# simonfuhrmann/mve

Hardware: AMD Instinct MI355X
Metric: depth-maps/sec (1920x1080, 20 views, scale=2) (higher is better)
Workload: dtype f32

## Files before the change

### mve_amd/csrc/dmrecon_device.hip

```cpp
#include <hip/hip_runtime.h>
#include <stdint.h>
#include <cstdlib>
#include <type_traits>

#include "dmrecon_types.h"
#include "dmrecon_device.h"

#define WAVE 64

#ifndef MI_FW
#define MI_FW 5
#endif
#define MI_HALF (MI_FW / 2)
#define MI_NS (MI_FW * MI_FW)
#define MI_MID (MI_NS / 2)
#define MI_STEP_SAMPLE (MI_NS > 12 ? 12 : MI_MID)
#define MI_CAT2(a, b) a##b
#define MI_CAT(a, b) MI_CAT2(a, b)
#define MI_FWNS MI_CAT(mi_fw, MI_FW)
#define MI_BULK_WAVES (MI_FW >= 7 ? 1 : MI_WAVES_PER_SIMD)
#ifdef MI_EMU_LIN48
#define MI_QUAD_WORDS 12
#elif defined(MI_QUAD_RECORDS)
#define MI_QUAD_WORDS 4
// ... 1884 lines not shown
#endif
struct XcdRange {
    unsigned per_x, base, j, jn;
    __device__ __forceinline__ explicit XcdRange(unsigned n_units, bool own_segment = false) {
        const unsigned nx = (gridDim.x % MI_XCDS == 0 && gridDim.x >= MI_XCDS) ? MI_XCDS : 1u;
        per_x = own_segment ? n_units : (n_units + nx - 1) / nx;
        base = own_segment ? 0u : (blockIdx.x % nx) * per_x; j = blockIdx.x / nx; jn = gridDim.x / nx;
    }
    __device__ __forceinline__ bool next(unsigned& unit) {
        if (j >= per_x) return false;
        unit = base + j; j += jn;
        return true;
    }
};

template <class L>
__device__ __forceinline__ void flush_counters(DevCounters* counters, int lane, unsigned n_eval, unsigned n_pass,
                                               unsigned n_patch, unsigned n_filled, unsigned err, int kind) {
    if (L::sub(lane) != 0) { n_eval = 0; n_pass = 0; }
    if (L::vslot(lane) != 0 || L::sub(lane) != 0) { n_patch = 0; n_filled = 0; }
    for (int off = 32; off > 0; off >>= 1) {
        n_eval += __shfl_down(n_eval, off);
        n_pass += __shfl_down(n_pass, off);
        n_patch += __shfl_down(n_patch, off);
        n_filled += __shfl_down(n_filled, off);
        err |= __shfl_down(err, off);
    }
    if (lane == 0) {
        if (n_eval) { atomicAdd(&counters->n_eval, (unsigned long long)n_eval); atomicAdd(&counters->k_eval[kind], (unsigned long long)n_eval); }
        if (n_pass) { atomicAdd(&counters->n_pass, (unsigned long long)n_pass); atomicAdd(&counters->k_pass[kind], (unsigned long long)n_pass);
                      atomicAdd(&counters->k_pass_exec[kind], (unsigned long long)n_pass); }
        if (n_patch) { atomicAdd(&counters->n_patch, (unsigned long long)n_patch); atomicAdd(&counters->k_patch[kind], (unsigned long long)n_patch); }
        if (n_filled) atomicAdd(&counters->n_filled, (unsigned long long)n_filled);
        if (err) atomicOr(&counters->error_flags, err);
    }
}

template <class L, bool FAST, bool SINGLE = FAST, bool SEED = false>
__global__ __launch_bounds__(WAVE) __attribute__((amdgpu_waves_per_eu((L::LAT ? 2 : MI_BULK_WAVES), (L::LAT ? 2 : MI_WAVES_PER_SIMD)))) void k_optimize(OptArgs a) {
    static_assert(SINGLE || !FAST, "the FAST kernel runs one attempt per entry");
    static_assert(!SEED || (SINGLE && !FAST), "the seed launch is the single-attempt form of the general kernel");
    const int lane = threadIdx.x;
    const bool grid8 = gridDim.x % MI_XCDS == 0 && gridDim.x >= MI_XCDS;
    const unsigned seg_n = (a.follow_seg != 0u && grid8) ? MI_XCDS : 1u, seg = blockIdx.x % seg_n;
    const unsigned seg_in_n = (a.follow_seg_in != 0u && grid8) ? MI_XCDS : 1u, seg_in = blockIdx.x % seg_in_n;
    const unsigned n = a.follow_in ? a.follow_in_n[seg_in] : (a.n_work_ptr ? *a.n_work_ptr : a.n_work);
    if (!a.follow_in && (n < a.min_work || n >= a.max_work)) return;
    for (int i = lane; i < 256; i += WAVE) g_lut[i] = a.lut[i];
#ifdef MI_ACTIVITY
    if (lane < 2) g_act[lane] = 0;
// ... 131 lines not shown
        PatchResult r; unsigned ne = 0, np = 0;
        unsigned deferred = 0;
        optimize_patch<L, false, true>(job, a.st, a.views, x, y, hd, hi, hj, hv, lane, r, ne, np, err, a.counters, &deferred);
        if (L::sub(lane) != 0) { ne = 0; np = 0; }
        ne = patch_sum_u<L>(ne); np = patch_sum_u<L>(np);
        if (writer) n_exec += np;
        if (writer) {
            DevSpec o;
            o.conf = r.conf; o.depth = r.depth; o.dzI = r.dzI; o.dzJ = r.dzJ; o.nx = r.nx; o.ny = r.ny; o.nz = r.nz;
            o.views = r.views; o.views_hi = r.views_hi; o.iters = r.iters; o.bc = bc; o.own = own; o.n_eval = ne; o.n_pass = np;
            o.n_cand = n_cand; o.pad = (int32_t)deferred;
            *rec = o;
        }
    }
    for (int off = 32; off > 0; off >>= 1) { err |= __shfl_down(err, off); n_exec += __shfl_down(n_exec, off); }
    if (lane == 0 && err) atomicOr(&a.counters->error_flags, err);
    if (lane == 0 && n_exec) atomicAdd(&a.counters->k_pass_exec[MI_KIND_SPEC], (unsigned long long)n_exec);
}

#define MI_TAIL_WAVES 4
static_assert(MI_TAIL_WAVES <= MI_LAT_SLOTS, "the latency layout's LDS holds one patch per wavefront of a tail workgroup");
#ifndef MI_TAIL_SPEC_WAVES
#define MI_TAIL_SPEC_WAVES 2
#endif
struct TailArgs {
    OptArgs o;
    const DevEntry* prev_work;
    const DevResult* prev_results;
    unsigned* round_work;
};

struct Frozen { float conf; int upd; bool one; };
// ... 130 lines not shown
                o.accepted = 1; o.tried = done;
                a.results[e] = o;
                const bool one = me.one;
                float* dp = one ? job->depth : job->depth1; float* zp = one ? job->dz : job->dz1;
                float* cq = one ? job->conf : job->conf1; float* np = one ? job->normal : job->normal1;
                uint32_t* vp = one ? job->views : job->views1; int32_t* up = one ? job->upd : job->upd1;
                dp[q] = fin.depth; zp[2 * q] = fin.dzI; zp[2 * q + 1] = fin.dzJ;
                np[3 * q] = fin.nx; np[3 * q + 1] = fin.ny; np[3 * q + 2] = fin.nz;
                cq[q] = fin.conf; vp[q] = fin.views; up[q] = a.round;
                if (NV == 8) (one ? job->views_hi : job->views1_hi)[q] = fin.views_hi;
                if (own <= 0.f) { ++n_filled; atomicAdd(const_cast<uint32_t*>(&job->n_filled), 1u); }
            }
        }
        if (SPEC && !single) __syncthreads();
    }
    if (threadIdx.x == 0) {
        if (n_eval) { atomicAdd(&a.counters->n_eval, (unsigned long long)n_eval); atomicAdd(&a.counters->k_eval[MI_KIND_TAIL], (unsigned long long)n_eval); }
        if (n_pass) { atomicAdd(&a.counters->n_pass, (unsigned long long)n_pass); atomicAdd(&a.counters->k_pass[MI_KIND_TAIL], (unsigned long long)n_pass);
                      atomicAdd(&a.counters->k_pass_exec[MI_KIND_TAIL], (unsigned long long)n_pass); }
        if (n_patch) { atomicAdd(&a.counters->n_patch, (unsigned long long)n_patch); atomicAdd(&a.counters->k_patch[MI_KIND_TAIL], (unsigned long long)n_patch); }
        if (n_filled) atomicAdd(&a.counters->n_filled, (unsigned long long)n_filled);
    }
    for (int off = 32; off > 0; off >>= 1) err |= __shfl_down(err, off);
    if (lane == 0 && err) atomicOr(&a.counters->error_flags, err);
}



#ifndef MI_FRONT_WAVES
#define MI_FRONT_WAVES 8
#endif
#define MI_FRONT_QCAP 256
#define MI_FRONT_GRAN 12
static_assert(MI_FRONT_WAVES <= MI_LAT_SLOTS, "the latency layout's LDS holds one patch per wavefront of a front workgroup");
struct FrontArgs {
    OptArgs o;
    DevEntry* work[2];
// ... 367 lines not shown
        __hip_atomic_store(t.host_done + jobi, 1u, __ATOMIC_RELEASE, __HIP_MEMORY_SCOPE_SYSTEM);
    }
    if (tid == 0) {
        if (gave_up) {
            atomicMax(t.job_resume + jobi, ((unsigned long long)(unsigned)round << 32) | ((unsigned long long)n_prev << 1) | (unsigned long long)cur);
            atomicOr(&a.counters->error_flags, 32u);
        } else if (n_prev == 0 || abort || g_fcnt[6] != 0) atomicMax(t.job_resume + jobi, MI_FRONT_DONE);
    }
    if (member != 0) { n_eval = 0; n_pass = 0; n_patch = 0; }
    for (int off2 = 32; off2 > 0; off2 >>= 1) {
        n_eval += __shfl_down(n_eval, off2); n_pass += __shfl_down(n_pass, off2);
        n_patch += __shfl_down(n_patch, off2); n_filled += __shfl_down(n_filled, off2);
        err |= __shfl_down(err, off2); st_att += __shfl_down(st_att, off2);
    }
    if (lane == 0) {
        if (n_eval) { atomicAdd(&a.counters->n_eval, (unsigned long long)n_eval); atomicAdd(&a.counters->k_eval[MI_KIND_FRONT], (unsigned long long)n_eval); }
        if (n_pass) { atomicAdd(&a.counters->n_pass, (unsigned long long)n_pass); atomicAdd(&a.counters->k_pass[MI_KIND_FRONT], (unsigned long long)n_pass);
                      atomicAdd(&a.counters->k_pass_exec[MI_KIND_FRONT], (unsigned long long)n_pass); }
        if (n_patch) { atomicAdd(&a.counters->n_patch, (unsigned long long)n_patch); atomicAdd(&a.counters->k_patch[MI_KIND_FRONT], (unsigned long long)n_patch); }
        if (n_filled) atomicAdd(&a.counters->n_filled, (unsigned long long)n_filled);
        if (err) atomicOr(&a.counters->error_flags, err);
        if (st_att) atomicAdd(&t.job_stats[4 * jobi + 1], st_att);
    }
    if (tid == 0 && member == 0) {
        atomicAdd(&t.job_stats[4 * jobi], st_rounds - (gave_up ? 1u : 0u)); atomicAdd(&t.job_stats[4 * jobi + 2], st_list - (gave_up ? n_prev : 0u));
        atomicAdd(&t.job_stats[4 * jobi + 3], (unsigned)(wall_clock64() - t0));
        if (n_prev != 0 && !abort && round >= t.max_rounds) atomicOr(&a.counters->error_flags, 8u);
    }
}

struct FrontSplitArgs {
    const DevEntry* work; const DevResult* results; const unsigned* n_ptr;
    DevEntry* owork; DevResult* oresults; const unsigned* job_off; unsigned* job_count;
};
__global__ __launch_bounds__(256) void k_front_split(FrontSplitArgs a) {
    const unsigned n = *a.n_ptr;
// ... 302 lines not shown
        filled += (unsigned)__popcll(__ballot(newly));
        unsigned long long todo = __ballot(newly);
        while (todo) {
            const int leader = __ffsll((long long)todo) - 1;
            const int lj = __shfl(myjob, leader);
            const unsigned long long same = __ballot(newly && myjob == lj);
            if ((int)(threadIdx.x & 63) == leader) atomicAdd(const_cast<uint32_t*>(&a.jobs[lj].n_filled), (unsigned)__popcll(same));
            todo &= ~same;
        }
    }
    __shared__ unsigned s_filled;
    if (threadIdx.x == 0) s_filled = 0;
    __syncthreads();
    if (filled && (threadIdx.x & 63) == 0) atomicAdd(&s_filled, filled);
    __syncthreads();
    if (threadIdx.x == 0 && s_filled) atomicAdd(&a.counters->n_filled, (unsigned long long)s_filled);
}

__global__ __launch_bounds__(256) void k_apply_spec(ApplyArgs a) {
    const unsigned n = a.n_work_ptr ? *a.n_work_ptr : a.n_work;
    if (n < a.min_work || n >= a.max_work) return;
    unsigned filled = 0, n_eval = 0, n_pass = 0, n_patch = 0;
    const unsigned n_items = *a.n_items;
    for (unsigned base = blockIdx.x * 256; base < n_items; base += gridDim.x * 256) {
        const unsigned i = base + threadIdx.x;
        bool newly = false;
        int myjob = -1;
        const unsigned item = i < n_items ? a.items[i] : 1u;
        if ((item & 3u) == 0u) {
            const unsigned e = item >> 2;
            const DevSpec* rec = a.spec + i;
// ... 42 lines not shown
        }
    }
    __shared__ unsigned s_red[4];
    if (threadIdx.x < 4) s_red[threadIdx.x] = 0;
    __syncthreads();
    for (int off = 32; off > 0; off >>= 1) {
        n_eval += __shfl_down(n_eval, off); n_pass += __shfl_down(n_pass, off); n_patch += __shfl_down(n_patch, off);
    }
    if ((threadIdx.x & 63) == 0) {
        if (filled) atomicAdd(&s_red[0], filled);
        if (n_eval) atomicAdd(&s_red[1], n_eval);
        if (n_pass) atomicAdd(&s_red[2], n_pass);
        if (n_patch) atomicAdd(&s_red[3], n_patch);
    }
    __syncthreads();
    if (threadIdx.x == 0) {
        if (s_red[0]) atomicAdd(&a.counters->n_filled, (unsigned long long)s_red[0]);
        if (s_red[1]) { atomicAdd(&a.counters->n_eval, (unsigned long long)s_red[1]); atomicAdd(&a.counters->k_eval[MI_KIND_SPEC], (unsigned long long)s_red[1]); }
        if (s_red[2]) { atomicAdd(&a.counters->n_pass, (unsigned long long)s_red[2]); atomicAdd(&a.counters->k_pass[MI_KIND_SPEC], (unsigned long long)s_red[2]); }
        if (s_red[3]) { atomicAdd(&a.counters->n_patch, (unsigned long long)s_red[3]); atomicAdd(&a.counters->k_patch[MI_KIND_SPEC], (unsigned long long)s_red[3]); }
    }
}

__global__ __launch_bounds__(256) void k_apply_seeds(ApplyArgs a) {
    const unsigned e = blockIdx.x * 256 + threadIdx.x;
    bool newly = false, okseed = false;
    if (e < a.n_work) {
        const DevResult r = a.results[e];
        const float c1 = a.seed_reopt ? __uint_as_float((unsigned)r.accepted) : r.conf;
        if (c1 > 0.f) {
            const DevEntry ent = a.work[e];
            const DevJob* job = a.jobs + ent.job;
            const int pix = (ent.xy >> 16) * job->w + (ent.xy & 0xFFFF);
            const unsigned long long key = ((unsigned long long)__float_as_uint(c1) << 32) | (0xFFFFFFFFu - e);
            unsigned long long* slot = a.seed_keys + a.key_off[ent.job] + pix;
            if (a.phase == 0) {
                atomicMax(slot, key);
                okseed = true;
            } else if (*slot == key) {
                newly = job->conf[pix] <= 0.f;
                write_pixel(job, pix, r, a.seed_reopt ? (r.tried ? 1 : 0) : a.round, e);
                if (a.seed_reopt && a.seed_count) atomicAdd(a.seed_count + ent.job, 1u);
                if (newly) atomicAdd(const_cast<uint32_t*>(&job->n_filled), 1u);
            }
        }
    }
    const unsigned long long m = __ballot(newly);
    if (m && (threadIdx.x & 63) == __ffsll((long long)m) - 1)
        atomicAdd(&a.counters->n_filled, (unsigned long long)__popcll(m));
    const unsigned long long m2 = __ballot(okseed);
    if (m2 && (threadIdx.x & 63) == __ffsll((long long)m2) - 1)
        atomicAdd(&a.counters->n_seeds_ok, (unsigned long long)__popcll(m2));
}


__global__ __launch_bounds__(256) void k_unpack_jobs(const uint32_t* __restrict__ packed, unsigned words_per_job, uint32_t* __restrict__ jobs, unsigned words_per_slot) {
    const unsigned j = blockIdx.y;
    for (unsigned w = blockIdx.x * 256 + threadIdx.x; w < words_per_job; w += gridDim.x * 256)
        jobs[(size_t)j * words_per_slot + w] = packed[(size_t)j * words_per_job + w];
}

__global__ __launch_bounds__(256) void k_pack_rgba(const uint8_t* __restrict__ src, uint32_t* __restrict__ dst,
                                                  int n, int channels) {
    const int i = blockIdx.x * 256 + threadIdx.x;
    if (i >= n) return;
    uint32_t r, g, b;
    if (channels <= 2) { r = g = b = src[(size_t)i * channels]; }
// ... 33 lines not shown
        }
    const float q0 = v0 / wsum, q1 = v1 / wsum, q2 = v2 / wsum;
    const uint32_t b0 = (uint32_t)(q0 > 0.f ? floorf(q0 + 0.5f) : 0.f);
    const uint32_t b1 = (uint32_t)(q1 > 0.f ? floorf(q1 + 0.5f) : 0.f);
    const uint32_t b2 = (uint32_t)(q2 > 0.f ? floorf(q2 + 0.5f) : 0.f);
    dst[(size_t)y * ow + x] = (b0 & 255u) | ((b1 & 255u) << 8) | ((b2 & 255u) << 16) | 0xFF000000u;
}

__global__ __launch_bounds__(256) void k_round_report(const unsigned* __restrict__ a, int n_a, const unsigned* __restrict__ b, int n_b,
                                                       const DevCounters* __restrict__ counters, const DevJob* __restrict__ jobs, int n_jobs,
                                                       unsigned* __restrict__ out_rw, unsigned* __restrict__ out_hc, unsigned* __restrict__ out_dyn,
                                                       const unsigned* __restrict__ view_count) {
    const int tid = (int)threadIdx.x;
    for (int i = tid; i < n_a; i += 256) out_rw[i] = a[i];
    for (int i = tid; i < n_b; i += 256) out_rw[n_a + i] = b[i];
    if (tid < (int)(sizeof(DevCounters) / sizeof(unsigned))) out_hc[tid] = reinterpret_cast<const unsigned*>(counters)[tid];
    static_assert(offsetof(DevJob, n_filled) == offsetof(DevJob, flags) + 4, "flags and n_filled are read as a pair");
    for (int j = tid; j < n_jobs; j += 256) {
        out_dyn[3 * j] = (unsigned)jobs[j].flags;
        out_dyn[3 * j + 1] = jobs[j].n_filled;
        out_dyn[3 * j + 2] = view_count ? view_count[j] : 0u;
    }
}

__global__ __launch_bounds__(256) void k_quadify(const uint32_t* __restrict__ src, u32x4* __restrict__ dst, int w, int h) {
    const int i = blockIdx.x * 256 + threadIdx.x;
    if (i >= w * h) return;
    const int y = i / w, x = i - y * w;
    const int x1 = x + 1 < w ? x + 1 : x, y1 = y + 1 < h ? y + 1 : y;
    u32x4 o;
    o.x = src[y * w + x]; o.y = src[y * w + x1]; o.z = src[y1 * w + x]; o.w = src[y1 * w + x1];
// ... 79 lines not shown

#if MI_FW == 5
unsigned long long* mi_debug_tbuf = nullptr;
#endif

static void launch_optimize(hipStream_t s, int lanes_per_view, unsigned grid_blocks, const DevJob* jobs, const DevView* views,
                        const float* lut, const DevSettings& st, const DevEntry* work, const DevHyp* hyp,
                        DevResult* results, const unsigned* n_work_ptr, unsigned n_work, unsigned min_work,
                        unsigned max_work, int round, DevCounters* counters, const unsigned* follow_in,
                        const unsigned* follow_in_n, unsigned* follow_out, unsigned* follow_out_n, unsigned follow_seg,
                        unsigned follow_seg_in, unsigned long long* follow_mask) {
    if (grid_blocks == 0) return;
    grid_blocks = (grid_blocks + MI_XCDS - 1) / MI_XCDS * MI_XCDS;
    OptArgs a;
    a.follow_seg = follow_seg; a.follow_seg_in = follow_seg_in; a.follow_mask = follow_mask;
    { const char* e = getenv("MI_DMRECON_DEBUG_SCRAMBLE"); a.scramble = (e && follow_in == nullptr && hyp == nullptr) ? (unsigned)atoi(e) : 0u; }
    a.jobs = jobs; a.views = views; a.lut = lut; a.st = st; a.work = work; a.hyp = hyp; a.results = results;
    a.n_work_ptr = n_work_ptr; a.n_work = n_work; a.min_work = min_work; a.max_work = max_work;
    a.round = round; a.counters = counters; a.tbuf = mi_debug_tbuf;
    a.max_attempts = (follow_out || follow_mask) ? 1 : 4; a.follow_in = follow_in; a.follow_in_n = follow_in_n;
    a.follow_out = follow_out; a.follow_out_n = follow_out_n;
    const bool lat = lanes_per_view != 1 && lanes_per_view != 2, eight = st.K > 4;
    if (st.K > 8) {
        if (lat) return;
        const unsigned ncc16 = (unsigned)(Lay<1, 16>::PATCHES * st.ncc_stride * sizeof(float));
        const bool single16 = hyp != nullptr || follow_out != nullptr;
        if (hyp != nullptr && st.seed_reopt) hipLaunchKernelGGL((k_optimize<Lay<1, 16>, false, true, true>), dim3(grid_blocks), dim3(WAVE), ncc16, s, a);
        else if (single16) hipLaunchKernelGGL((k_optimize<Lay<1, 16>, false, true>), dim3(grid_blocks), dim3(WAVE), ncc16, s, a);
        else hipLaunchKernelGGL((k_optimize<Lay<1, 16>, false>), dim3(grid_blocks), dim3(WAVE), ncc16, s, a);
        return;
    }
// ... 223 lines not shown
```

### mve_amd/csrc/dmrecon_host.cpp

```cpp
#include "../../include/mi_dmrecon.h"
#include "../../include/mi_dmrecon_debug.h"

#include <hip/hip_runtime.h>
#include <omp.h>
#include <fcntl.h>
#include <sys/file.h>
#include <sys/stat.h>
#include <unistd.h>
#include <cctype>
#include <cerrno>

#include <algorithm>
#include <atomic>
#include <condition_variable>
#include <thread>
#include <chrono>
#include <cmath>
#include <cstdarg>
#include <cstdio>
#include <cstdlib>
#include <cstring>
#include <ctime>
#include <limits>
#include <immintrin.h>
// ... 147 lines not shown
        return 0;
    }
    void release() { if (p) (void)hipFree(p); p = nullptr; cap = 0; }
};

#define MI_TAIL_CHUNK 32
struct TailPoll { unsigned rw[MI_TAIL_CHUNK]; DevCounters hc; };
#define MI_MAX_DEVICES 64
std::atomic<int> g_active_calls[MI_MAX_DEVICES];
std::atomic<int> g_inject_footprint(-1);
#define MI_MERGE_SMALL_CALL 48
#define MI_MERGE_WINDOW_US 1000
#define MI_MERGE_WINDOW_BIG_US 3000
#define MI_SINGLE_FOLLOW 4
#define MI_FAST_FOLLOW 0
#define MI_FOLLOW_LISTS 64
#define MI_ONE_LAUNCH_MAX 100000u
#define MI_SPEC_ROUNDS 400000u
#define MI_VIEW_HANDOVER 320u
#define MI_TEAM_WAIT_US 20000u
#define MI_FRONT_MIN_CAP 256
#define MI_FRONT_PER_TEAM_WG 64
struct ActiveCall {
    int dev;
    explicit ActiveCall(int d) : dev(d >= 0 && d < MI_MAX_DEVICES ? d : -1) { if (dev >= 0) g_active_calls[dev].fetch_add(1); }
    ~ActiveCall() { if (dev >= 0) g_active_calls[dev].fetch_sub(1); }
    bool alone() const { return dev < 0 || g_active_calls[dev].load() <= 1; }
    int count() const { return dev < 0 ? 1 : g_active_calls[dev].load(); }
};

struct JobHost {
// ... 161 lines not shown
        d_views.release();
        d_geom_sees.release(); d_geom_valid.release(); d_geom_zcam.release(); d_geom_plx.release();
        d_geom_fpos.release(); d_geom_inv0.release();
        if (d_lut) (void)hipFree(d_lut);
    }
};

struct mi_dmrecon_ctx {
    int device = 0;
    int n_cus = 64;
    double wall_clock_khz = 100000.0;
    hipStream_t stream = nullptr;
    hipStream_t stream2 = nullptr;
    std::shared_ptr<SceneStore> sc;
    DevCounters* d_counters = nullptr;
    DevBuf<uint8_t> d_stage;
    DevBuf<uint8_t> d_stage2;
    int stage_flip = 0;
    BatchScratch bs;
};

namespace {

int sync_views(mi_dmrecon_ctx* c) {
    std::lock_guard<std::mutex> lock(c->sc->mu);
    if (!c->sc->views_dirty) return 0;
    std::vector<DevView> hv(c->sc->views.size());
    for (size_t i = 0; i < c->sc->views.size(); ++i) {
        HostView const& v = c->sc->views[i];
        DevView& d = hv[i];
// ... 826 lines not shown
static int create_streams(mi_dmrecon_ctx* c) {
    HIP_TRY(hipStreamCreateWithFlags(&c->stream, hipStreamNonBlocking));
    int prio_least = 0, prio_greatest = 0;
    if (hipDeviceGetStreamPriorityRange(&prio_least, &prio_greatest) != hipSuccess) { prio_least = prio_greatest = 0; (void)hipGetLastError(); }
    if (prio_greatest != prio_least) HIP_TRY(hipStreamCreateWithPriority(&c->stream2, hipStreamNonBlocking, prio_greatest));
    else HIP_TRY(hipStreamCreateWithFlags(&c->stream2, hipStreamNonBlocking));
    int cus = 0;
    if (hipDeviceGetAttribute(&cus, hipDeviceAttributeMultiprocessorCount, c->device) == hipSuccess && cus > 0) c->n_cus = cus;
    int khz = 0;
    if (hipDeviceGetAttribute(&khz, hipDeviceAttributeWallClockRate, c->device) == hipSuccess && khz > 0) c->wall_clock_khz = (double)khz;
    else (void)hipGetLastError();
    return 0;
}

static int warm_streams(mi_dmrecon_ctx* c) {
    HIP_TRY(hipMemsetAsync(c->d_counters, 0, sizeof(DevCounters), c->stream));
    HIP_TRY(hipMemsetAsync(c->d_counters, 0, sizeof(DevCounters), c->stream2));
    HIP_TRY(hipStreamSynchronize(c->stream));
    HIP_TRY(hipStreamSynchronize(c->stream2));
    return 0;
}

int mi_dmrecon_ctx_create(int device, mi_dmrecon_ctx** out) {
    if (!out) return fail(MI_DMRECON_EINVAL, "null out pointer");
    int n = mi_dmrecon_device_count();
    if (n <= 0) return fail(MI_DMRECON_EDEVICE, "no HIP device available (this library has no CPU path)");
    if (device < 0 || device >= n) return fail(MI_DMRECON_EINVAL, "device %d out of range (0..%d)", device, n - 1);
    HIP_TRY(hipSetDevice(device));
    mi_dmrecon_ctx* c = new mi_dmrecon_ctx;
    c->device = device;
    c->sc = std::make_shared<SceneStore>();
    c->sc->device = device;
    if (int rc = create_streams(c)) return rc;
    float lut[256];
    for (int i = 0; i < 256; ++i) {
        double x = i / 255.0;
        lut[i] = (float)((i <= 0.04045 * 255.0) ? x / 12.92 : std::pow((x + 0.055) / 1.055, 2.4));
    }
    lut[255] = 1.0f;
    HIP_TRY(hipMalloc((void**)&c->sc->d_lut, sizeof(lut)));
    HIP_TRY(hipMemcpy(c->sc->d_lut, lut, sizeof(lut), hipMemcpyHostToDevice));
    HIP_TRY(hipMalloc((void**)&c->d_counters, sizeof(DevCounters)));
    if (int rc = warm_streams(c)) return rc;
    *out = c;
    return 0;
}

void mi_dmrecon_ctx_destroy(mi_dmrecon_ctx* c) {
    if (!c) return;
    (void)hipSetDevice(c->device);
    (void)wait_stream(c->stream);
    if (c->stream2) (void)wait_stream(c->stream2);
    c->bs.release();
    c->d_stage.release(); c->d_stage2.release();
    if (c->d_counters) (void)hipFree(c->d_counters);
    (void)hipStreamDestroy(c->stream);
    if (c->stream2) (void)hipStreamDestroy(c->stream2);
    delete c;
}

int mi_dmrecon_ctx_fork(mi_dmrecon_ctx* parent, mi_dmrecon_ctx** out) {
    if (!parent || !out) return fail(MI_DMRECON_EINVAL, "null argument");
    HIP_TRY(hipSetDevice(parent->device));
    mi_dmrecon_ctx* c = new mi_dmrecon_ctx;
    c->device = parent->device;
    c->sc = parent->sc;
    if (int rc = create_streams(c)) return rc;
    HIP_TRY(hipMalloc((void**)&c->d_counters, sizeof(DevCounters)));
    if (int rc = warm_streams(c)) return rc;
    *out = c;
    return 0;
}

void* mi_dmrecon_host_alloc(size_t bytes) {
    void* p = nullptr;
    if (hipHostMalloc(&p, bytes, hipHostMallocDefault) != hipSuccess) { fail(MI_DMRECON_EDEVICE, "hipHostMalloc(%zu) failed", bytes); return nullptr; }
    return p;
}
void mi_dmrecon_host_free(void* p) { if (p) (void)hipHostFree(p); }

void* mi_dmrecon_ctx_stream(mi_dmrecon_ctx* c) { return c ? (void*)c->stream : nullptr; }

static size_t host_view_set_camera(HostView& v, const mi_dmrecon_camera* cam, int32_t width, int32_t height) {
// ... 405 lines not shown
        const size_t jb = job_bytes;
#pragma omp parallel for schedule(static) num_threads(n_threads) if (n_threads > 1)
        for (int j = 0; j < nj; ++j) {
            std::memcpy(hu + up_jobs + (size_t)j * jb, &dj[j], job_prefix_bytes(dj[j].n_global));
            const size_t n = jobs[j].seeds.size();
            if (n) {
                std::memcpy(hu + up_seeds + seed_off[j] * sizeof(DevEntry), jobs[j].seeds.data(), n * sizeof(DevEntry));
                std::memcpy(hu + up_hyps + seed_off[j] * sizeof(DevHyp), jobs[j].seed_hyp.data(), n * sizeof(DevHyp));
            }
        }
    }
    mark("  upload: staging");
    if (c->bs.d_jobs_packed.reserve(((size_t)nj * job_bytes + 3) / 4)) return fail(MI_DMRECON_EDEVICE, "hipMalloc(jobs) failed");
    HIP_TRY(hipMemcpyAsync(c->bs.d_jobs_packed.p, c->bs.h_up + up_jobs, (size_t)nj * job_bytes, hipMemcpyHostToDevice, S));
    mi_launch_unpack_jobs(S, c->bs.d_jobs_packed.p, (unsigned)(job_bytes / 4), c->bs.d_jobs.p, nj);
    HIP_TRY(hipMemsetAsync(c->d_counters, 0, sizeof(DevCounters), S));
    if (c->bs.d_hyp.reserve(std::max<size_t>(n_seeds_total, 1)) || c->bs.d_keyoff.reserve(nj)
        || c->bs.d_round_work.reserve(MI_MAX_ROUNDS) || c->bs.d_round_work_t.reserve(MI_MAX_ROUNDS) || c->bs.d_round_items.reserve(MI_MAX_ROUNDS)
        || c->bs.d_follow_cnt.reserve(MI_FOLLOW_LISTS * MI_MAX_ROUNDS) || c->bs.d_view.reserve(4 * (size_t)nj)
        || c->bs.d_front.reserve(7 * (size_t)nj) || c->bs.d_front_resume.reserve(2 * (size_t)nj))
        return fail(MI_DMRECON_EDEVICE, "hipMalloc(work lists) failed");
    HIP_TRY(hipMemsetAsync(c->bs.d_round_work.p, 0, MI_MAX_ROUNDS * sizeof(unsigned), S));
    HIP_TRY(hipMemsetAsync(c->bs.d_round_work_t.p, 0, MI_MAX_ROUNDS * sizeof(unsigned), S));
    HIP_TRY(hipMemsetAsync(c->bs.d_round_items.p, 0, MI_MAX_ROUNDS * sizeof(unsigned), S));
    if (const char* e = std::getenv("MI_DMRECON_VIEW_HANDOVER")) handover = (unsigned)std::max(0L, std::atol(e));
    host_rounds_only = [] { const char* e = std::getenv("MI_DMRECON_HOST_ROUNDS"); return e && std::atoi(e) != 0; }();
    if (st->nrReconNeighbors > 8) handover = 0;
    HIP_TRY(hipMemsetAsync(c->bs.d_view.p, 0, 4 * (size_t)nj * sizeof(unsigned), S));
    if (handover < 1000000000u) HIP_TRY(hipMemsetAsync(c->bs.d_view.p, 0xFF, (size_t)nj * sizeof(unsigned), S));
    HIP_TRY(hipMemsetAsync(c->bs.d_follow_cnt.p, 0, MI_FOLLOW_LISTS * MI_MAX_ROUNDS * sizeof(unsigned), S));
    HIP_TRY(hipMemcpyAsync(c->bs.d_keyoff.p, c->bs.h_up + up_keyoff, nj * sizeof(unsigned), hipMemcpyHostToDevice, S));
// ... 75 lines not shown
    struct Pending { int round; size_t ev_thr, ev_lat; };
    Pending pend[2]; int n_pend = 0;
    bool stop = false;
    const bool SEED_REOPT = seed_mode == 1;
    auto enqueue = [&](int r) -> int {
        const bool spec = SPEC_MAX > 0 && known_thr < SPEC_MAX;
        const bool self = SEED_REOPT && r == 1;
        DevSettings ds = this->ds;
        ds.self_round = self ? 1 : 0;
        ev.begin(S, EventLog::SWEEP, 0);
        D->generate(S, c->bs.d_jobs.p, nj, max_tiles, c->bs.d_work.p, c->bs.d_work2.p, c->bs.d_round_work_t.p, c->bs.d_round_work.p,
                    d_vcount, d_vmode, handover, r, spec ? c->bs.d_follow.p : nullptr, c->bs.d_round_items.p, self ? 1 : 0);
        ev.end(S);
        const unsigned* n_thr_p = c->bs.d_round_work_t.p + r; const unsigned* n_lat_p = c->bs.d_round_work.p + r;
        const unsigned est = std::max(2u * known_thr, 65536u);
        const unsigned waves = (est + ppw - 1) / ppw;
        const bool any_lat = !wide && (r >= 2 || handover >= 1000000000u);
        ev.begin(S, EventLog::BULK, 0);
        const size_t ev_thr = ev.items.size() - 1;
        size_t ev_lat = (size_t)-1;
        unsigned* fcnt = c->bs.d_follow_cnt.p + MI_FOLLOW_LISTS * (size_t)r;
        const unsigned plain_min = spec ? spec_cap : 0u;
        const bool need_plain = !spec || 16ull * (unsigned long long)known_thr >= (unsigned long long)spec_cap;
        if (spec) {
            const unsigned quads = std::min(std::max(3u * known_thr, 16384u), 4u * spec_cap);
            D->optimize_spec(S, (quads + ppw - 1) / ppw, c->bs.d_jobs.p, c->sc->d_views.p, c->sc->d_lut, ds, c->bs.d_work.p, c->bs.d_spec.p,
                             c->bs.d_follow.p, c->bs.d_round_items.p + r, n_thr_p, 0u, 0u, spec_cap, r, c->d_counters);
        }
        if (!need_plain) { }
        else if (known_thr < ONE_LAUNCH_MAX)
            D->optimize(S, 1, spec ? std::max(1u, waves / 2) : waves, c->bs.d_jobs.p, c->sc->d_views.p, c->sc->d_lut, ds, c->bs.d_work.p, nullptr, c->bs.d_results.p, n_thr_p,
                        0u, plain_min, 0xFFFFFFFFu, r, c->d_counters, nullptr, nullptr, nullptr, nullptr, 0u, 0u, nullptr);
        else {
            const bool segs = [] { const char* e = std::getenv("MI_DMRECON_FOLLOW_SEGMENTS"); return !e || std::atoi(e) != 0; }();
            const unsigned fseg_full = (unsigned)((total_px + MI_FOLLOW_SEGS - 1) / MI_FOLLOW_SEGS) + 64u;
            const unsigned fseg = segs ? fseg_full : 0u;
            const size_t fstride = (size_t)fseg_full * MI_FOLLOW_SEGS;
            unsigned* fl[5] = {c->bs.d_follow.p, c->bs.d_follow.p + fstride, c->bs.d_follow.p + 2 * fstride, c->bs.d_follow.p + 3 * fstride, c->bs.d_follow.p};
            const bool ordered = SINGLE_FOLLOW && !std::getenv("MI_DMRECON_DEBUG_SCRAMBLE")
                && [] { const char* e = std::getenv("MI_DMRECON_FOLLOW_ORDERED"); return !e || std::atoi(e) != 0; }();
            if (ordered && (c->bs.d_fmask.reserve(total_px / ppw + 4096) || c->bs.d_fblk.reserve(1024)))
                return fail(MI_DMRECON_EDEVICE, "hipMalloc(follow-up masks) failed");
            D->optimize(S, 1, waves, c->bs.d_jobs.p, c->sc->d_views.p, c->sc->d_lut, ds, c->bs.d_work.p, nullptr, c->bs.d_results.p, n_thr_p,
                        0u, plain_min, 0xFFFFFFFFu, r, c->d_counters, nullptr, nullptr, ordered ? nullptr : fl[0], fcnt, fseg, 0u, ordered ? c->bs.d_fmask.p : nullptr);
            if (ordered) mi_launch_follow_compact(S, c->bs.d_fmask.p, n_thr_p, plain_min, 0xFFFFFFFFu, ppw, 64u / ppw, c->bs.d_fblk.p, fl[0], fcnt);
            if (SINGLE_FOLLOW) {
                unsigned div = 4;
                const int n_single = SINGLE_FOLLOW >= 4 ? 4 : std::max(1, SINGLE_FOLLOW);
                for (int k = 0; k < n_single; ++k, div *= 4) {
                    D->optimize(S, k < FAST_FOLLOW ? 2 : 1, std::max(64u, waves / div), c->bs.d_jobs.p, c->sc->d_views.p, c->sc->d_lut, ds, c->bs.d_work.p, nullptr,
                                c->bs.d_results.p, n_thr_p, 0u, 0u, 0xFFFFFFFFu, r, c->d_counters, fl[k], fcnt + MI_FOLLOW_SEGS * k, fl[k + 1], fcnt + MI_FOLLOW_SEGS * (k + 1), fseg,
                                (k == 0 && ordered) ? 0u : fseg, nullptr);
                    ++n_launch;
                }
// ... 66 lines not shown
        while (n_pend > 1 || (stop && n_pend > 0)) {
            const int r = retire();
            if (r < 0) return r;
            if (r == 1) {
                while (n_pend > 0) { HIP_TRY(wait_event(c->bs.poll_ev[pend[0].round & 1])); pend[0] = pend[1]; --n_pend; }
                round = last_seen; done = true;
                return 0;
            }
            if (n_alive == 0) { HIP_TRY(wait_stream(S)); return 0; }
            if (last_thr == 0 && !host_rounds_only) stop = true;
        }
    }
    if (stop) {
        if (last_thr != 0) return fail(MI_DMRECON_EDEVICE, "internal: throughput entries after the hand-over");
        tail_known = last_lat;
        HIP_TRY(hipMemcpyAsync(&c->bs.h_poll[2].hc, c->d_counters, sizeof(hc), hipMemcpyDeviceToHost, S));
        have_handover = true;
        to_tail = true;
        return 0;
    }
    if (n_alive > 0) truncated = true;
    return 0;
}

int BatchRun::tail_rounds(bool& to_front) {
    to_front = false;
    sparse_r0 = round;
    static const unsigned SPEC_MAX = [] { const char* e = std::getenv("MI_DMRECON_SPECULATE"); return e ? (unsigned)std::atoi(e) : 1024u; }();
    const ActiveCall& active = *active_call;
    plan_front_team();
    const unsigned FRONT_PER_VIEW = [&] {
// ... 274 lines not shown
                    if (!streamed[j] && __atomic_load_n(&h_done[j], __ATOMIC_ACQUIRE) != 0u) {
                        if (int rc = (sparse && snapped[j]) ? emit_view(j) : stream_view(j)) return rc;
                        if (!over) ++n_streamed_early;
                        if (trace) fprintf(stderr, "[mi_dmrecon] view %d streamed back at %.3f ms of the front phase (%s)\n", jobs[j].ref_view, now_ms() - t_mark, over ? "kernel over" : "kernel running");
                    }
                if (sparse) scatter_emitted(false);
                if (over || n_streamed == nj) break;
                if (g_patient_waits) std::this_thread::sleep_for(std::chrono::microseconds(50));
                else for (int k = 0; k < 200; ++k) cpu_relax();
            }
        }
        if (h_done) {
            mi_launch_round_report(S, d_stats, 4 * nj, nullptr, 0, c->d_counters, c->bs.d_jobs.p, nj, h_done + nj, &P.hc, dyn_of(0), nullptr);
            HIP_TRY(hipGetLastError());
        } else {
            HIP_TRY(hipMemcpyAsync(&P.hc, c->d_counters, sizeof(hc), hipMemcpyDeviceToHost, S));
            HIP_TRY(read_dyn(0));
            HIP_TRY(hipMemcpyAsync(front_stats.data(), d_stats, 4 * (size_t)nj * sizeof(unsigned), hipMemcpyDeviceToHost, S));
        }
        HIP_TRY(wait_stream(S));
        if (sparse) {
            HIP_TRY(wait_stream(c->stream2));
            scatter_emitted(true);
            if (sparse_overflow)
                for (int j = 0; j < nj; ++j) if (snapped[j] && streamed[j] == 1) { streamed[j] = 0; --n_streamed; snapped[j] = 0; }
            if (trace) fprintf(stderr, "[mi_dmrecon] maps: snapshot of %d views at the hand-over (round %d) + %u changed pixels%s\n",
                               (int)emit_order.size(), sparse_r0, sparse_done_end, sparse_overflow ? " -- list overflow, full copies instead" : "");
        }
        if (h_done) std::memcpy(front_stats.data(), h_done + nj, 4 * (size_t)nj * sizeof(unsigned));
        hc = P.hc;
        token.reset();
// ... 475 lines not shown
        }
        for (; cnt < 16; ++cnt) packed[cnt >> 3] |= (unsigned long long)MI_VIEW_NONE << (8 * (cnt & 7));
        hy[i].views = (uint32_t)packed[0]; hy[i].views_hi = (uint32_t)(packed[0] >> 32);
        if (nch == 16) { hyx[2 * (size_t)i] = (uint32_t)packed[1]; hyx[2 * (size_t)i + 1] = (uint32_t)(packed[1] >> 32); }
    }
    if (nch == 16) {
        uint32_t* d_hx = dj[0].results_x + 2 * std::max(total_px, (size_t)n);
        dj[0].hyp_x = d_hx;
        HIP_TRY(hipMemcpyAsync(d_hx, hyx.data(), 2 * (size_t)n * sizeof(uint32_t), hipMemcpyHostToDevice, c->stream));
    }
    if (c->bs.d_jobs.reserve(1) || c->bs.d_work.reserve(n) || c->bs.d_hyp.reserve(n) || c->bs.d_results.reserve(n))
        return fail(MI_DMRECON_EDEVICE, "hipMalloc failed");
    HIP_TRY(hipMemcpyAsync(c->bs.d_jobs.p, dj.data(), sizeof(DevJob), hipMemcpyHostToDevice, c->stream));
    HIP_TRY(hipMemcpyAsync(c->bs.d_work.p, ent.data(), n * sizeof(DevEntry), hipMemcpyHostToDevice, c->stream));
    HIP_TRY(hipMemcpyAsync(c->bs.d_hyp.p, hy.data(), n * sizeof(DevHyp), hipMemcpyHostToDevice, c->stream));
    HIP_TRY(hipMemsetAsync(c->d_counters, 0, sizeof(DevCounters), c->stream));
    const int lpv = lanes_per_view == 16 ? 16 : 1;
    if (lpv == 16 && st->nrReconNeighbors > 8)
        return fail(MI_DMRECON_EINVAL, "more than eight local views run in the throughput layout only (lanes_per_view = 1)");
    const unsigned ppw = lpv == 16 ? 1u : patches_per_wave(st);
    D.optimize(c->stream, lpv, ((unsigned)n + ppw - 1) / ppw, c->bs.d_jobs.p, c->sc->d_views.p, c->sc->d_lut, dev_settings(st),
               c->bs.d_work.p, c->bs.d_hyp.p, c->bs.d_results.p, nullptr, (unsigned)n, 0u, 0xFFFFFFFFu, 0, c->d_counters,
               nullptr, nullptr, nullptr, nullptr, 0u, 0u, nullptr);
    HIP_TRY(hipGetLastError());
    std::vector<DevResult> res(n); std::vector<uint32_t> resx(2 * (size_t)n, 0xFFFFFFFFu);
    HIP_TRY(hipMemcpyAsync(res.data(), c->bs.d_results.p, n * sizeof(DevResult), hipMemcpyDeviceToHost, c->stream));
    if (nch == 16) HIP_TRY(hipMemcpyAsync(resx.data(), dj[0].results_x, 2 * (size_t)n * sizeof(uint32_t), hipMemcpyDeviceToHost, c->stream));
    HIP_TRY(wait_stream(c->stream));
    for (int i = 0; i < n; ++i) {
        float* o = out + 8 * i;
        o[0] = res[i].conf; o[1] = res[i].depth; o[2] = res[i].dzI; o[3] = res[i].dzJ;
// ... 247 lines not shown
```

### mve_amd/csrc/dmrecon_types.h

```cpp
#ifndef MI_DMRECON_TYPES_H
#define MI_DMRECON_TYPES_H

#include <stdint.h>

#define MI_MAX_LEVELS 16
#define MI_MAX_GLOBAL 128
#define MI_AVAIL_WORDS (MI_MAX_GLOBAL / 64)
#define MI_MAX_LOCAL 16
#define MI_MAX_FW 7
#define MI_PATCHES_PER_WAVE 16
#define MI_VIEW_NONE 0xFFu
#define MI_MAX_ROUNDS 8192

struct DevLevel {
    float ax, ay, cx, cy;
    float inv0;
    int32_t w, h;
    uint32_t tex_off;
};

struct DevView {
    float cam_pos[3];
    float w2c[12];
    int32_t n_levels;
// ... 84 lines not shown
    int32_t n_cand;
    int32_t pad;
};

struct DevCounters {
    unsigned long long n_patch, n_eval, n_pass, n_filled, n_seeds_ok;
    unsigned long long n_stage;
    unsigned long long n_gather_pass;
    unsigned long long n_view_replaced;
    unsigned long long n_iter14;
    unsigned int error_flags;
    unsigned int pad;
    unsigned long long k_eval[8], k_pass[8], k_patch[8], k_pass_exec[8];
    unsigned long long clk_shader, clk_real;
};
enum { MI_KIND_FAST = 0, MI_KIND_FOLLOW = 1, MI_KIND_SEED = 2, MI_KIND_LOOP = 3, MI_KIND_SPEC = 4, MI_KIND_LAT = 5, MI_KIND_TAIL = 6, MI_KIND_FRONT = 7 };

#endif
```

Before: 1734.

## Stripe device counters across 64 slots and shrink bulk launch grid

Result: faster. 1999, median of 6 (+15.3%).

```diff
diff --git a/mve_amd/csrc/dmrecon_device.hip b/mve_amd/csrc/dmrecon_device.hip
--- a/mve_amd/csrc/dmrecon_device.hip
+++ b/mve_amd/csrc/dmrecon_device.hip
@@ -1922,6 +1922,20 @@
     }
 };
 
+__device__ __forceinline__ DevCounters* counter_stripe(DevCounters* counters) {
+    return &reinterpret_cast<DevCounterStripe*>(counters)[blockIdx.x % MI_COUNTER_STRIPES].c;
+}
+__device__ __forceinline__ void add_work_counts(DevCounters* counters, int kind, unsigned n_eval, unsigned n_pass, unsigned n_exec,
+                                                unsigned n_patch, unsigned n_filled, unsigned err) {
+    DevCounters* c = counter_stripe(counters);
+    if (n_eval) atomicAdd(&c->k_eval[kind], (unsigned long long)n_eval);
+    if (n_pass) atomicAdd(&c->k_pass[kind], (unsigned long long)n_pass);
+    if (n_exec) atomicAdd(&c->k_pass_exec[kind], (unsigned long long)n_exec);
+    if (n_patch) atomicAdd(&c->k_patch[kind], (unsigned long long)n_patch);
+    if (n_filled) atomicAdd(&c->n_filled, (unsigned long long)n_filled);
+    if (err) atomicOr(&counters->error_flags, err);
+}
+
 template <class L>
 __device__ __forceinline__ void flush_counters(DevCounters* counters, int lane, unsigned n_eval, unsigned n_pass,
                                                unsigned n_patch, unsigned n_filled, unsigned err, int kind) {
@@ -1934,14 +1948,7 @@
         n_filled += __shfl_down(n_filled, off);
         err |= __shfl_down(err, off);
     }
-    if (lane == 0) {
-        if (n_eval) { atomicAdd(&counters->n_eval, (unsigned long long)n_eval); atomicAdd(&counters->k_eval[kind], (unsigned long long)n_eval); }
-        if (n_pass) { atomicAdd(&counters->n_pass, (unsigned long long)n_pass); atomicAdd(&counters->k_pass[kind], (unsigned long long)n_pass);
-                      atomicAdd(&counters->k_pass_exec[kind], (unsigned long long)n_pass); }
-        if (n_patch) { atomicAdd(&counters->n_patch, (unsigned long long)n_patch); atomicAdd(&counters->k_patch[kind], (unsigned long long)n_patch); }
-        if (n_filled) atomicAdd(&counters->n_filled, (unsigned long long)n_filled);
-        if (err) atomicOr(&counters->error_flags, err);
-    }
+    if (lane == 0) add_work_counts(counters, kind, n_eval, n_pass, n_pass, n_patch, n_filled, err);
 }
 
 template <class L, bool FAST, bool SINGLE = FAST, bool SEED = false>
@@ -2103,8 +2110,7 @@
         }
     }
     for (int off = 32; off > 0; off >>= 1) { err |= __shfl_down(err, off); n_exec += __shfl_down(n_exec, off); }
-    if (lane == 0 && err) atomicOr(&a.counters->error_flags, err);
-    if (lane == 0 && n_exec) atomicAdd(&a.counters->k_pass_exec[MI_KIND_SPEC], (unsigned long long)n_exec);
+    if (lane == 0) add_work_counts(a.counters, MI_KIND_SPEC, 0u, 0u, n_exec, 0u, 0u, err);
 }
 
 #define MI_TAIL_WAVES 4
@@ -2265,13 +2271,7 @@
         }
         if (SPEC && !single) __syncthreads();
     }
-    if (threadIdx.x == 0) {
-        if (n_eval) { atomicAdd(&a.counters->n_eval, (unsigned long long)n_eval); atomicAdd(&a.counters->k_eval[MI_KIND_TAIL], (unsigned long long)n_eval); }
-        if (n_pass) { atomicAdd(&a.counters->n_pass, (unsigned long long)n_pass); atomicAdd(&a.counters->k_pass[MI_KIND_TAIL], (unsigned long long)n_pass);
-                      atomicAdd(&a.counters->k_pass_exec[MI_KIND_TAIL], (unsigned long long)n_pass); }
-        if (n_patch) { atomicAdd(&a.counters->n_patch, (unsigned long long)n_patch); atomicAdd(&a.counters->k_patch[MI_KIND_TAIL], (unsigned long long)n_patch); }
-        if (n_filled) atomicAdd(&a.counters->n_filled, (unsigned long long)n_filled);
-    }
+    if (threadIdx.x == 0) add_work_counts(a.counters, MI_KIND_TAIL, n_eval, n_pass, n_pass, n_patch, n_filled, 0u);
     for (int off = 32; off > 0; off >>= 1) err |= __shfl_down(err, off);
     if (lane == 0 && err) atomicOr(&a.counters->error_flags, err);
 }
@@ -2669,12 +2669,7 @@
         err |= __shfl_down(err, off2); st_att += __shfl_down(st_att, off2);
     }
     if (lane == 0) {
-        if (n_eval) { atomicAdd(&a.counters->n_eval, (unsigned long long)n_eval); atomicAdd(&a.counters->k_eval[MI_KIND_FRONT], (unsigned long long)n_eval); }
-        if (n_pass) { atomicAdd(&a.counters->n_pass, (unsigned long long)n_pass); atomicAdd(&a.counters->k_pass[MI_KIND_FRONT], (unsigned long long)n_pass);
-                      atomicAdd(&a.counters->k_pass_exec[MI_KIND_FRONT], (unsigned long long)n_pass); }
-        if (n_patch) { atomicAdd(&a.counters->n_patch, (unsigned long long)n_patch); atomicAdd(&a.counters->k_patch[MI_KIND_FRONT], (unsigned long long)n_patch); }
-        if (n_filled) atomicAdd(&a.counters->n_filled, (unsigned long long)n_filled);
-        if (err) atomicOr(&a.counters->error_flags, err);
+        add_work_counts(a.counters, MI_KIND_FRONT, n_eval, n_pass, n_pass, n_patch, n_filled, err);
         if (st_att) atomicAdd(&t.job_stats[4 * jobi + 1], st_att);
     }
     if (tid == 0 && member == 0) {
@@ -3007,7 +3002,7 @@
     __syncthreads();
     if (filled && (threadIdx.x & 63) == 0) atomicAdd(&s_filled, filled);
     __syncthreads();
-    if (threadIdx.x == 0 && s_filled) atomicAdd(&a.counters->n_filled, (unsigned long long)s_filled);
+    if (threadIdx.x == 0) add_work_counts(a.counters, 0, 0u, 0u, 0u, 0u, s_filled, 0u);
 }
 
 __global__ __launch_bounds__(256) void k_apply_spec(ApplyArgs a) {
@@ -3080,12 +3075,7 @@
         if (n_patch) atomicAdd(&s_red[3], n_patch);
     }
     __syncthreads();
-    if (threadIdx.x == 0) {
-        if (s_red[0]) atomicAdd(&a.counters->n_filled, (unsigned long long)s_red[0]);
-        if (s_red[1]) { atomicAdd(&a.counters->n_eval, (unsigned long long)s_red[1]); atomicAdd(&a.counters->k_eval[MI_KIND_SPEC], (unsigned long long)s_red[1]); }
-        if (s_red[2]) { atomicAdd(&a.counters->n_pass, (unsigned long long)s_red[2]); atomicAdd(&a.counters->k_pass[MI_KIND_SPEC], (unsigned long long)s_red[2]); }
-        if (s_red[3]) { atomicAdd(&a.counters->n_patch, (unsigned long long)s_red[3]); atomicAdd(&a.counters->k_patch[MI_KIND_SPEC], (unsigned long long)s_red[3]); }
-    }
+    if (threadIdx.x == 0) add_work_counts(a.counters, MI_KIND_SPEC, s_red[1], s_red[2], 0u, s_red[3], s_red[0], 0u);
 }
 
 __global__ __launch_bounds__(256) void k_apply_seeds(ApplyArgs a) {
@@ -3113,10 +3103,10 @@
     }
     const unsigned long long m = __ballot(newly);
     if (m && (threadIdx.x & 63) == __ffsll((long long)m) - 1)
-        atomicAdd(&a.counters->n_filled, (unsigned long long)__popcll(m));
+        add_work_counts(a.counters, MI_KIND_SEED, 0u, 0u, 0u, 0u, (unsigned)__popcll(m), 0u);
     const unsigned long long m2 = __ballot(okseed);
     if (m2 && (threadIdx.x & 63) == __ffsll((long long)m2) - 1)
-        atomicAdd(&a.counters->n_seeds_ok, (unsigned long long)__popcll(m2));
+        atomicAdd(&counter_stripe(a.counters)->n_seeds_ok, (unsigned long long)__popcll(m2));
 }
 
 
@@ -3180,7 +3170,27 @@
     const int tid = (int)threadIdx.x;
     for (int i = tid; i < n_a; i += 256) out_rw[i] = a[i];
     for (int i = tid; i < n_b; i += 256) out_rw[n_a + i] = b[i];
-    if (tid < (int)(sizeof(DevCounters) / sizeof(unsigned))) out_hc[tid] = reinterpret_cast<const unsigned*>(counters)[tid];
+    constexpr int CW = (int)(sizeof(DevCounters) / sizeof(unsigned long long));
+    static_assert(sizeof(DevCounters) % sizeof(unsigned long long) == 0 && CW <= 256 && offsetof(DevCounters, error_flags) % 8 == 0, "summed as 64-bit words");
+    __shared__ unsigned long long s_cnt[CW];
+    if (tid < CW) {
+        const bool flags = tid == (int)(offsetof(DevCounters, error_flags) / 8);
+        unsigned long long v = 0;
+        for (int s = 0; s < MI_COUNTER_STRIPES; ++s) {
+            const unsigned long long w = reinterpret_cast<const unsigned long long*>(&reinterpret_cast<const DevCounterStripe*>(counters)[s].c)[tid];
+            v = flags ? (v | w) : (v + w);
+        }
+        s_cnt[tid] = v;
+    }
+    __syncthreads();
+    if (tid < CW) {
+        unsigned long long v = s_cnt[tid];
+        const int k0 = tid == (int)(offsetof(DevCounters, n_eval) / 8) ? (int)(offsetof(DevCounters, k_eval) / 8)
+                     : tid == (int)(offsetof(DevCounters, n_pass) / 8) ? (int)(offsetof(DevCounters, k_pass) / 8)
+                     : tid == (int)(offsetof(DevCounters, n_patch) / 8) ? (int)(offsetof(DevCounters, k_patch) / 8) : -1;
+        if (k0 >= 0) for (int k = 0; k < 8; ++k) v += s_cnt[k0 + k];
+        out_hc[2 * tid] = (unsigned)v; out_hc[2 * tid + 1] = (unsigned)(v >> 32);
+    }
     static_assert(offsetof(DevJob, n_filled) == offsetof(DevJob, flags) + 4, "flags and n_filled are read as a pair");
     for (int j = tid; j < n_jobs; j += 256) {
         out_dyn[3 * j] = (unsigned)jobs[j].flags;
@@ -3290,7 +3300,8 @@
     grid_blocks = (grid_blocks + MI_XCDS - 1) / MI_XCDS * MI_XCDS;
     OptArgs a;
     a.follow_seg = follow_seg; a.follow_seg_in = follow_seg_in; a.follow_mask = follow_mask;
-    { const char* e = getenv("MI_DMRECON_DEBUG_SCRAMBLE"); a.scramble = (e && follow_in == nullptr && hyp == nullptr) ? (unsigned)atoi(e) : 0u; }
+    static const unsigned scramble_env = [] { const char* e = getenv("MI_DMRECON_DEBUG_SCRAMBLE"); return e ? (unsigned)atoi(e) : 0u; }();
+    a.scramble = (follow_in == nullptr && hyp == nullptr) ? scramble_env : 0u;
     a.jobs = jobs; a.views = views; a.lut = lut; a.st = st; a.work = work; a.hyp = hyp; a.results = results;
     a.n_work_ptr = n_work_ptr; a.n_work = n_work; a.min_work = min_work; a.max_work = max_work;
     a.round = round; a.counters = counters; a.tbuf = mi_debug_tbuf;
diff --git a/mve_amd/csrc/dmrecon_host.cpp b/mve_amd/csrc/dmrecon_host.cpp
--- a/mve_amd/csrc/dmrecon_host.cpp
+++ b/mve_amd/csrc/dmrecon_host.cpp
@@ -185,7 +185,9 @@
 #define MI_MERGE_WINDOW_BIG_US 3000
 #define MI_SINGLE_FOLLOW 4
 #define MI_FAST_FOLLOW 0
-#define MI_FOLLOW_LISTS 64
+#define MI_BULK_UNITS 4
+#define MI_BULK_MIN_WAVES 16384u
+#define MI_FOLLOW_LISTS (5 * MI_FOLLOW_SEGS)
 #define MI_ONE_LAUNCH_MAX 100000u
 #define MI_SPEC_ROUNDS 400000u
 #define MI_VIEW_HANDOVER 320u
@@ -377,6 +379,7 @@
     hipStream_t stream2 = nullptr;
     std::shared_ptr<SceneStore> sc;
     DevCounters* d_counters = nullptr;
+    int bulk_units = MI_BULK_UNITS;
     DevBuf<uint8_t> d_stage;
     DevBuf<uint8_t> d_stage2;
     int stage_flip = 0;
@@ -1233,8 +1236,8 @@
 }
 
 static int warm_streams(mi_dmrecon_ctx* c) {
-    HIP_TRY(hipMemsetAsync(c->d_counters, 0, sizeof(DevCounters), c->stream));
-    HIP_TRY(hipMemsetAsync(c->d_counters, 0, sizeof(DevCounters), c->stream2));
+    HIP_TRY(hipMemsetAsync(c->d_counters, 0, MI_COUNTER_BYTES, c->stream));
+    HIP_TRY(hipMemsetAsync(c->d_counters, 0, MI_COUNTER_BYTES, c->stream2));
     HIP_TRY(hipStreamSynchronize(c->stream));
     HIP_TRY(hipStreamSynchronize(c->stream2));
     return 0;
@@ -1250,6 +1253,7 @@
     c->device = device;
     c->sc = std::make_shared<SceneStore>();
     c->sc->device = device;
+    if (const char* e = std::getenv("MI_DMRECON_BULK_UNITS")) c->bulk_units = std::max(1, std::min(16, std::atoi(e)));
     if (int rc = create_streams(c)) return rc;
     float lut[256];
     for (int i = 0; i < 256; ++i) {
@@ -1259,7 +1263,7 @@
     lut[255] = 1.0f;
     HIP_TRY(hipMalloc((void**)&c->sc->d_lut, sizeof(lut)));
     HIP_TRY(hipMemcpy(c->sc->d_lut, lut, sizeof(lut), hipMemcpyHostToDevice));
-    HIP_TRY(hipMalloc((void**)&c->d_counters, sizeof(DevCounters)));
+    HIP_TRY(hipMalloc((void**)&c->d_counters, MI_COUNTER_BYTES));
     if (int rc = warm_streams(c)) return rc;
     *out = c;
     return 0;
@@ -1284,8 +1288,9 @@
     mi_dmrecon_ctx* c = new mi_dmrecon_ctx;
     c->device = parent->device;
     c->sc = parent->sc;
+    c->bulk_units = parent->bulk_units;
     if (int rc = create_streams(c)) return rc;
-    HIP_TRY(hipMalloc((void**)&c->d_counters, sizeof(DevCounters)));
+    HIP_TRY(hipMalloc((void**)&c->d_counters, MI_COUNTER_BYTES));
     if (int rc = warm_streams(c)) return rc;
     *out = c;
     return 0;
@@ -1721,7 +1726,7 @@
     if (c->bs.d_jobs_packed.reserve(((size_t)nj * job_bytes + 3) / 4)) return fail(MI_DMRECON_EDEVICE, "hipMalloc(jobs) failed");
     HIP_TRY(hipMemcpyAsync(c->bs.d_jobs_packed.p, c->bs.h_up + up_jobs, (size_t)nj * job_bytes, hipMemcpyHostToDevice, S));
     mi_launch_unpack_jobs(S, c->bs.d_jobs_packed.p, (unsigned)(job_bytes / 4), c->bs.d_jobs.p, nj);
-    HIP_TRY(hipMemsetAsync(c->d_counters, 0, sizeof(DevCounters), S));
+    HIP_TRY(hipMemsetAsync(c->d_counters, 0, MI_COUNTER_BYTES, S));
     if (c->bs.d_hyp.reserve(std::max<size_t>(n_seeds_total, 1)) || c->bs.d_keyoff.reserve(nj)
         || c->bs.d_round_work.reserve(MI_MAX_ROUNDS) || c->bs.d_round_work_t.reserve(MI_MAX_ROUNDS) || c->bs.d_round_items.reserve(MI_MAX_ROUNDS)
         || c->bs.d_follow_cnt.reserve(MI_FOLLOW_LISTS * MI_MAX_ROUNDS) || c->bs.d_view.reserve(4 * (size_t)nj)
@@ -1827,7 +1832,8 @@
         ev.end(S);
         const unsigned* n_thr_p = c->bs.d_round_work_t.p + r; const unsigned* n_lat_p = c->bs.d_round_work.p + r;
         const unsigned est = std::max(2u * known_thr, 65536u);
-        const unsigned waves = (est + ppw - 1) / ppw;
+        const unsigned waves1 = (est + ppw - 1) / ppw;
+        const unsigned waves = std::max((waves1 + (unsigned)c->bulk_units - 1) / (unsigned)c->bulk_units, std::min(waves1, MI_BULK_MIN_WAVES));
         const bool any_lat = !wide && (r >= 2 || handover >= 1000000000u);
         ev.begin(S, EventLog::BULK, 0);
         const size_t ev_thr = ev.items.size() - 1;
@@ -1850,7 +1856,8 @@
             const unsigned fseg = segs ? fseg_full : 0u;
             const size_t fstride = (size_t)fseg_full * MI_FOLLOW_SEGS;
             unsigned* fl[5] = {c->bs.d_follow.p, c->bs.d_follow.p + fstride, c->bs.d_follow.p + 2 * fstride, c->bs.d_follow.p + 3 * fstride, c->bs.d_follow.p};
-            const bool ordered = SINGLE_FOLLOW && !std::getenv("MI_DMRECON_DEBUG_SCRAMBLE")
+            static const bool scrambled = std::getenv("MI_DMRECON_DEBUG_SCRAMBLE") != nullptr;
+            const bool ordered = SINGLE_FOLLOW && !scrambled
                 && [] { const char* e = std::getenv("MI_DMRECON_FOLLOW_ORDERED"); return !e || std::atoi(e) != 0; }();
             if (ordered && (c->bs.d_fmask.reserve(total_px / ppw + 4096) || c->bs.d_fblk.reserve(1024)))
                 return fail(MI_DMRECON_EDEVICE, "hipMalloc(follow-up masks) failed");
@@ -1947,7 +1954,8 @@
     if (stop) {
         if (last_thr != 0) return fail(MI_DMRECON_EDEVICE, "internal: throughput entries after the hand-over");
         tail_known = last_lat;
-        HIP_TRY(hipMemcpyAsync(&c->bs.h_poll[2].hc, c->d_counters, sizeof(hc), hipMemcpyDeviceToHost, S));
+        mi_launch_round_report(S, nullptr, 0, nullptr, 0, c->d_counters, c->bs.d_jobs.p, 0, c->bs.h_poll[2].rw, &c->bs.h_poll[2].hc, nullptr, nullptr);
+        HIP_TRY(hipGetLastError());
         have_handover = true;
         to_tail = true;
         return 0;
@@ -2252,7 +2260,8 @@
             mi_launch_round_report(S, d_stats, 4 * nj, nullptr, 0, c->d_counters, c->bs.d_jobs.p, nj, h_done + nj, &P.hc, dyn_of(0), nullptr);
             HIP_TRY(hipGetLastError());
         } else {
-            HIP_TRY(hipMemcpyAsync(&P.hc, c->d_counters, sizeof(hc), hipMemcpyDeviceToHost, S));
+            mi_launch_round_report(S, nullptr, 0, nullptr, 0, c->d_counters, c->bs.d_jobs.p, 0, P.rw, &P.hc, nullptr, nullptr);
+            HIP_TRY(hipGetLastError());
             HIP_TRY(read_dyn(0));
             HIP_TRY(hipMemcpyAsync(front_stats.data(), d_stats, 4 * (size_t)nj * sizeof(unsigned), hipMemcpyDeviceToHost, S));
         }
@@ -2758,7 +2767,7 @@
     HIP_TRY(hipMemcpyAsync(c->bs.d_jobs.p, dj.data(), sizeof(DevJob), hipMemcpyHostToDevice, c->stream));
     HIP_TRY(hipMemcpyAsync(c->bs.d_work.p, ent.data(), n * sizeof(DevEntry), hipMemcpyHostToDevice, c->stream));
     HIP_TRY(hipMemcpyAsync(c->bs.d_hyp.p, hy.data(), n * sizeof(DevHyp), hipMemcpyHostToDevice, c->stream));
-    HIP_TRY(hipMemsetAsync(c->d_counters, 0, sizeof(DevCounters), c->stream));
+    HIP_TRY(hipMemsetAsync(c->d_counters, 0, MI_COUNTER_BYTES, c->stream));
     const int lpv = lanes_per_view == 16 ? 16 : 1;
     if (lpv == 16 && st->nrReconNeighbors > 8)
         return fail(MI_DMRECON_EINVAL, "more than eight local views run in the throughput layout only (lanes_per_view = 1)");
diff --git a/mve_amd/csrc/dmrecon_types.h b/mve_amd/csrc/dmrecon_types.h
--- a/mve_amd/csrc/dmrecon_types.h
+++ b/mve_amd/csrc/dmrecon_types.h
@@ -122,6 +122,9 @@
     unsigned long long k_eval[8], k_pass[8], k_patch[8], k_pass_exec[8];
     unsigned long long clk_shader, clk_real;
 };
+#define MI_COUNTER_STRIPES 64
+struct alignas(128) DevCounterStripe { DevCounters c; };
+#define MI_COUNTER_BYTES (MI_COUNTER_STRIPES * sizeof(DevCounterStripe))
 enum { MI_KIND_FAST = 0, MI_KIND_FOLLOW = 1, MI_KIND_SEED = 2, MI_KIND_LOOP = 3, MI_KIND_SPEC = 4, MI_KIND_LAT = 5, MI_KIND_TAIL = 6, MI_KIND_FRONT = 7 };
 
 #endif
```
